# Lainshower/debiasing-multi-modal

Measured on AMD Instinct MI355X. Metric: images/sec (embed+adapter step), CLIP-RN50 224px bs=1024, higher is better.
Workload: dtype f32; 1 GPU; CLIP-RN50 224px encode_image + adapter(1024-128-1024) CE/SGD step, 1024 images/GPU, global batch 1024 (the metric's configuration, CLIP-RN50 224px bs=1024 on one GPU); global_batch=1024, batch_per_gpu=1024, parallelism=dp1, collective=none

## Files before the change

debiasing-multi-modal_amd/_lib.py:

```python
import ctypes
import glob
import os
import subprocess
from ctypes import c_float, c_int, c_int64, c_size_t, c_void_p

_HERE = os.path.dirname(os.path.abspath(__file__))
CSRC = os.path.join(_HERE, "csrc")
LIB_PATH = os.environ.get("DBMM_LIB") or os.path.join(_HERE, "libdbmm_hip.so")
INCLUDE = os.path.join(os.path.dirname(_HERE), "include")

_lib = None


def sources():
    return sorted(glob.glob(os.path.join(CSRC, "*.hip")))


KERNEL_SOURCES = (
    ("igemm_", ("igemm_f32.hip", "igemm_epilogue.inc", "common.h")),
    ("bottleneck_chain_kernel", ("bottleneck_chain.hip", "common.h")),
    ("bottleneck_chain8_kernel", ("bottleneck_chain8.hip", "common.h")),
    ("conv3x3_c32_kernel", ("conv_patch.hip", "common.h")),
    ("gemm_pair_8ph_kernel", ("gemm_pair_8ph.hip", "common.h")),
    ("conv3x3_halo8", ("conv3x3_halo8.hip", "conv3x3_halo8_epilogue.inc", "common.h")),
# ... 82 lines not shown
    "dbmm_bottleneck_chain_x2": [_P, _P, _P, _I, _P, _P, _P, _P, _P, _P, _P, _I, _P, _P, _P, _P, _L, _L, _L, _L, _L, _L, _P],
    "dbmm_bottleneck_chain_dual_x2": [_P, _P, _P, _I, _P, _P, _P, _P, _P, _P, _P, _P, _P, _I, _P, _P, _P, _P, _L, _L, _L, _L, _L, _P],
    "dbmm_gemm_f16": [_P, _L, _P, _L, _P, _P, _L, _P, _L, _L, _L, _L, _I, _P],
    "dbmm_gemm_f16_ws": [_P, _L, _P, _L, _P, _P, _L, _P, _L, _L, _L, _L, _I, _P, _Z, _P],
    "dbmm_mha_core_f16": [_P, _P, _L, _L, _L, _L, _I, _P],
    "dbmm_layernorm_f16": [_P, _L, _P, _P, _P, _L, _L, _L, _F, _P],
    "dbmm_conv1x1_bn_act_f16": [_P, _P, _P, _P, _P, _P, _L, _L, _L, _I, _P],
    "dbmm_conv1x1_bn_act_f16_ws": [_P, _P, _P, _P, _P, _P, _L, _L, _L, _I, _P, _Z, _P],
    "dbmm_conv1x1_dual_bn_act_f16": [_P, _P, _P, _P, _P, _P, _P, _P, _L, _L, _L, _L, _I, _P],
    "dbmm_bottleneck_chain_f16": [_P, _P, _P, _P, _P, _P, _P, _P, _P, _P, _L, _L, _L, _L, _P],
    "dbmm_bottleneck_chain_pool_f16": [_P, _P, _P, _P, _P, _P, _P, _P, _P, _P, _P, _L, _L, _L, _L, _L, _L, _P],
    "dbmm_bottleneck_chain_dual_f16": [_P, _P, _P, _P, _P, _P, _P, _P, _P, _P, _P, _P, _L, _L, _L, _L, _L, _P],
    "dbmm_conv3x3_bn_relu_f16": [_P, _P, _P, _P, _P, _L, _L, _L, _L, _L, _I, _P],
    "dbmm_conv_stem_s2_f16": [_P, _I, _P, _P, _P, _L, _L, _L, _L, _P],
    "dbmm_conv1x1_res_pool_f16": [_P, _P, _P, _P, _P, _P, _P, _L, _L, _L, _L, _L, _P],
    "dbmm_conv_stem_s2_bn_f16": [_P, _I, _P, _P, _P, _P, _L, _L, _L, _L, _P],
    "dbmm_avgpool2_f16": [_P, _P, _L, _L, _L, _L, _P],
    "dbmm_im2col_patch_f16": [_P, _I, _P, _L, _L, _L, _L, _P],
    "dbmm_vit_tokens_f16": [_P, _P, _P, _P, _L, _L, _L, _P],
    "dbmm_embed_gather_f16": [_P, _P, _P, _P, _L, _L, _L, _L, _P],
    "dbmm_gather_eot_f16": [_P, _P, _P, _L, _L, _L, _P],
    "dbmm_cast_f32_f16": [_P, _P, _L, _P],
    "dbmm_conv3x3_c32_bn_relu_x2": [_P, _P, _P, _I, _P, _P, _P, _P, _L, _L, _L, _L, _L, _I, _P],
    "dbmm_bottleneck_block_chain_x2": [_P, _P, _P, _I, _P, _P, _P, _I, _P, _P, _P, _P, _P, _P, _P, _P, _P, _P, _I, _P, _P, _P, _P,
                                       _L, _L, _L, _L, _L, _L, _P],
    "dbmm_gemm_bias_act_x3": [_P, _L, _P, _P, _L, _P, _P, _L, _P, _L, _L, _L, _L, _F, _I, _P, _Z, _P],
    "dbmm_gemm_batched": [_P, _L, _L, _I, _P, _L, _L, _I, _P, _L, _P, _L, _L, _L, _L, _L, _L, _F, _I, _P],
    "dbmm_gemm_pair_8ph": [_P, _L, _P, _P, _I, _L, _P, _P, _P, _L, _P, _L, _P, _L, _L, _L, _F, _I, _P],
    "dbmm_conv_stem_s2": [_P, _P, _P, _P, _P, _L, _L, _L, _L, _P],
    "dbmm_avgpool2d": [_P, _P, _L, _L, _L, _L, _L, _P],
    "dbmm_workspace_bytes_attnpool": [_L, _L, _L],
    "dbmm_attnpool": [_P, _P, _P, _P, _P, _P, _P, _P, _P, _L, _L, _L, _L, _L, _P, _Z, _P],
    "dbmm_attnpool_x": [_P, _I, _P, _P, _P, _P, _P, _P, _P, _P, _L, _L, _L, _L, _L, _P, _Z, _P],
    "dbmm_layernorm": [_P, _L, _P, _P, _P, _L, _L, _L, _F, _P, _P],
    "dbmm_mha_core": [_P, _P, _L, _L, _L, _L, _I, _P],
    "dbmm_mha_core_x2": [_P, _P, _P, _L, _L, _L, _L, _I, _P],
    "dbmm_embed_gather": [_P, _P, _P, _P, _L, _L, _L, _L, _P],
    "dbmm_im2col_patch": [_P, _P, _P, _L, _L, _L, _P],
    "dbmm_vit_tokens": [_P, _P, _P, _P, _L, _L, _L, _P],
    "dbmm_gather_eot": [_P, _P, _P, _L, _L, _L, _P],
    "dbmm_bn1d_stats": [_P, _L, _L, _F, _F, _P, _P, _P, _P, _P, _P],
    "dbmm_bn1d_relu": [_P, _P, _P, _P, _P, _P, _L, _L, _I, _F, _P],
    "dbmm_adapter_fwd": [_P] * 15 + [_L, _L, _L, _I, _F, _F, _P],
    "dbmm_workspace_bytes_adapter_bwd": [_L, _L, _L],
    "dbmm_adapter_bwd": [_P] * 15 + [_L, _L, _L, _P, _Z, _P],
    "dbmm_text_colnorm": [_P, _P, _L, _L, _P],
# ... 93 lines not shown
```

debiasing-multi-modal_amd/clip/model.py:

```python
import os
import re
from collections import OrderedDict
from typing import Tuple, Union

import numpy as np
import torch
from torch import nn

from .. import ops



class _ConvW(nn.Module):
    def __init__(self, cin, cout, k):
        super().__init__()
        self.weight = nn.Parameter(torch.empty(cout, cin, k, k))


class _BNParams(nn.Module):
    def __init__(self, c):
        super().__init__()
        self.weight = nn.Parameter(torch.ones(c))
        self.bias = nn.Parameter(torch.zeros(c))
        self.register_buffer("running_mean", torch.zeros(c))
# ... 50 lines not shown
        super().__init__()
        self.positional_embedding = nn.Parameter(torch.randn(spacial_dim ** 2 + 1, embed_dim) / embed_dim ** 0.5)
        self.k_proj = _LinearW(embed_dim, embed_dim)
        self.q_proj = _LinearW(embed_dim, embed_dim)
        self.v_proj = _LinearW(embed_dim, embed_dim)
        self.c_proj = _LinearW(embed_dim, output_dim or embed_dim)
        self.num_heads = num_heads


def _fold_bn(conv_w, bn):
    s = bn.weight.double() / torch.sqrt(bn.running_var.double() + bn.eps)
    w = conv_w.double() * s.reshape(-1, 1, 1, 1)
    b = bn.bias.double() - bn.running_mean.double() * s
    return w, b


def _conv_bn(conv, bn):
    w, b = _fold_bn(conv.weight, bn)
    scale = bn.weight.detach().double() / torch.sqrt(bn.running_var.detach().double() + bn.eps)
    return _pack_conv(w, b, raw=conv.weight.detach().float(), scale=scale)


_PLAN_OPTIONS = {"conv_split": ("f16", ("f16", "bf16", "off")), "conv_k_order": ("chunk32", ("chunk32", "tap")),
                 "fuse_ds": (1, (0, 1)), "fuse_chain": (1, (0, 1)), "fuse_conv2": (1, (0, 1)), "seam_pool": (2, (0, 1, 2))}
_opt = {}
_opt_version = [0]


def set_plan_option(name, value):
    default, allowed = _PLAN_OPTIONS[name]
    if isinstance(default, int):
        value = int(value)
    if value not in allowed:
        raise ValueError(f"plan option {name}: {value!r} not in {allowed}")
    old = _opt.get(name, default)
    _opt[name] = value
    _opt_version[0] += 1
    return old


def plan_option(name):
    return _opt[name]


for _name in _PLAN_OPTIONS:
    set_plan_option(_name, os.environ.get("DBMM_" + _name.upper(), _PLAN_OPTIONS[_name][0]))

# ... 188 lines not shown
        out = ops.attnpool(x, a["pos"], a["wq"], a["bq"], a["wkv"], a["bkv"], a["wc"], a["bc"], self.attnpool.num_heads)
        out = out.to(torch.float16)
        return (out, stages) if return_stages else out

    def rounds_fp32_images_itself(self):
        return (self.conv1.weight.dtype == torch.float16 and self._f16_eligible()
                and all(b.stride in (1, 2) for li in (1, 2, 3, 4) for b in getattr(self, f"layer{li}")))

    @torch.no_grad()
    def forward(self, x, return_stages=False):
        if self.conv1.weight.dtype == torch.float16:
            if self._f16_eligible() and all(b.stride in (1, 2) for li in (1, 2, 3, 4) for b in getattr(self, f"layer{li}")):
                return self.forward_f16(x, return_stages)
            if not return_stages:
                return self.forward(x, return_stages=True)[0].to(torch.float16)
        if self._plan is not None and self._plan_key != self._param_key():
            self._plan = None
        P = self._plan or self._compile()
        x = x.float().contiguous()
        n_slots = 3 + 4 * len(P["blocks"])
        amax = torch.zeros(n_slots, device=x.device, dtype=torch.float32)
        slot = [1]
        track = _opt["conv_split"] == "f16"
        x = ops.conv_stem_s2(x, *P["stem1"], y_absmax=amax[0:1] if track else None)

        def conv(t, t_am, c, res, k, pad, act, pool=1, keep_full=False):
            y_am = amax[slot[0]:slot[0] + 1] if track else None; slot[0] += 1
            y = ops.conv_bn_act(t, c["w"], c["b"], res, k, k, 1, pad, act, c["wl"], w_planes=c["p3"],
                                w_planes_f16=c["ph"], w_exp=c["we"], x_absmax=t_am, y_absmax=y_am, out_scale=c["sc"],
                                pool=pool, keep_full=keep_full)
            return y, y_am

        x, am = conv(x, amax[0:1] if track else None, P["stem2"], None, 3, 1, ops.ACT_RELU)
        x, am = conv(x, am, P["stem3"], None, 3, 1, ops.ACT_RELU, pool=2)
        stages = {"stem": x}
        blocks = P["blocks"]
        x_pooled = None
        y1_next = None
        bi = 0
        for li in (1, 2, 3, 4):
            for _ in getattr(self, f"layer{li}"):
                e = blocks[bi]; bi += 1
                if y1_next is not None:
                    (out, oam), y1_next = y1_next, None
                else:
                    out, oam = conv(x, am, e["c1"], None, 1, 0, ops.ACT_RELU)
                nxt = blocks[bi] if bi < len(blocks) else None
                if (e["stride"] == 1 and track and _opt["fuse_chain"] and _opt["fuse_conv2"] and nxt is not None and nxt["stride"] == 1
                        and all(c["sc"] is not None and c["ph"] is not None for c in (e["c2"], e["c3"], nxt["c1"]))
                        and ("ds" not in e or ("dual" in e and _opt["fuse_ds"]))):
                    ndsl = 3 if "ds" in e else 2
                    x_am, y1_am = amax[slot[0] + 1:slot[0] + 2], amax[slot[0] + ndsl:slot[0] + ndsl + 1]
                    dual = dict(a2=x, a2_absmax=am, ds=e["ds"], ratio=e["dual"]["ratio"], bias=e["dual"]["bias"]) if "ds" in e else None
                    r = ops.bottleneck_block_chain(out, oam, e["c2"], e["c3"], nxt["c1"], residual=None if dual else x, dual=dual,
                                                   x_absmax=x_am, y1n_absmax=y1_am)
                    if r is not None:
# ... 343 lines not shown
```

debiasing-multi-modal_amd/csrc/common.h:

```cpp
#pragma once
#include <hip/hip_runtime.h>
#include <stdint.h>
#include <type_traits>
#include "../../include/dbmm.h"

typedef float f32x4 __attribute__((ext_vector_type(4)));
typedef float f32x16 __attribute__((ext_vector_type(16)));

#define DBMM_CHECK_LAUNCH()                      \
    do {                                         \
        hipError_t e__ = hipGetLastError();      \
        if (e__ != hipSuccess) return (int)e__;  \
    } while (0)

enum DbmmOpt {
    OPT_IGEMM_EPI_DIRECT, OPT_IGEMM_FAST, OPT_IGEMM_STREAMK, OPT_IGEMM_X3, OPT_IGEMM_X2, OPT_IGEMM_X2_BK, OPT_IGEMM_BK,
    OPT_IGEMM_HALO, OPT_IGEMM_HALO_POOL, OPT_IGEMM_BN256, OPT_IGEMM_BN256_KXK, OPT_GEMM_8PH, OPT_F16_8PH, OPT_F16_BN256,
    OPT_STEM_MFMA, OPT_MHA_VALU, OPT_CONV_PATCH, OPT_MHA_X2, OPT_ADAPTER_STEP_FUSED, OPT_CONV1X1_STREAM, OPT_CONV1X1_8PH, OPT_CHAIN8, OPT_CONV1X1_BN256, OPT_TAIL_SPLIT, OPT_HALO8, OPT_DUAL_8PH, OPT_MHA_SHORT, OPT_F16_CONV_8PH, OPT_CONV1X1_RES_STREAM, OPT_LINEAR_STEP_ONE_LAUNCH_MAX_B, DBMM_OPT_COUNT
};
int dbmm_opt(int id);

int dbmm_conv3x3_halo8(const float* x, const float* x_absmax, const void* w_plane_f16, int w_exp, const float* out_scale, const float* bias,
                       float* y, float* y_absmax, int64_t B, int64_t H, int64_t W, int64_t Cin, int64_t Cout, int act, int pool, int split,
                       void* workspace, size_t workspace_bytes, void* stream);

int dbmm_gemm_pair_8ph_ws(const float* a, int64_t lda, const float* a_absmax, const void* w_plane_f16, int w_exp, int64_t ldw,
                          const float* out_scale, const float* bias, const float* residual, int64_t ldr, float* c, int64_t ldc,
                          float* c_absmax, int64_t M, int64_t N, int64_t K, float alpha, int act, void* workspace, size_t workspace_bytes, void* stream);
int dbmm_gemm_dual_pair_8ph(const float* a, int64_t lda, const float* a_absmax, const void* w_plane_f16, int w_exp, int64_t ldw, int64_t K,
                            const float* out_scale, const float* a2, int64_t lda2, const float* a2_absmax, const void* w2_plane_f16, int64_t ldw2,
                            int64_t K2, const float* ratio, const float* bias, float* c, int64_t ldc, float* c_absmax, int64_t M, int64_t N, int act,
                            void* stream);

static inline int dbmm_cut_slices(int rem, int trips) {
    if (rem <= 0 || rem > 128) return 0;
    int S = 256 / rem;
    S = S < trips ? S : trips;
    S = S < 16 ? S : 16;
    return S >= 2 ? S : 0;
}

// ... 26 lines not shown
```

debiasing-multi-modal_amd/csrc/conv_patch.hip:

```cpp
#include <stdlib.h>
#include "common.h"

namespace {

typedef _Float16 f16x8 __attribute__((ext_vector_type(8)));
typedef unsigned short u16;
typedef unsigned int u32x2 __attribute__((ext_vector_type(2)));
typedef unsigned int u32x4 __attribute__((ext_vector_type(4)));

constexpr unsigned OOR = 0x80000000u;
constexpr long long EXT_LIM = 0x7FFFFFF0LL;
constexpr int TR = 4, TC = 28;
constexpr int PR = TR + 2, PC = TC + 2, PPX = PR * PC;
constexpr int CIN = 32, KTOT = 9 * CIN;
constexpr int WROW = KTOT + 8;

struct PatchP {
    const float* x; const float* x_absmax;
    const u16* w; int w_exp; const float* sc; const float* bias;
    float* y; float* y_absmax;
    int B, H, W, tiles_w, tiles_h, n_tiles;
};

__device__ __forceinline__ int scale_exp(float amax) {
    const unsigned b = __float_as_uint(amax) & 0x7fffffffu;
    int s = b ? 13 - ((int)(b >> 23) - 127) : 0;
    return s < -60 ? -60 : (s > 60 ? 60 : s);
}
__device__ __forceinline__ float pow2f(int e) { return __uint_as_float((unsigned)(e + 127) << 23); }

__device__ __forceinline__ void split2h_pair(float x0, float x1, float sc, unsigned& hi, unsigned& lo) {
#if defined(__HIP_DEVICE_COMPILE__)
    asm("v_fma_mixlo_f16 %0, %1, %2, 0" : "=v"(hi) : "v"(x0), "v"(sc));
    asm("v_fma_mixhi_f16 %0, %1, %2, 0" : "+v"(hi) : "v"(x1), "v"(sc));
    asm("v_fma_mixlo_f16 %0, %1, %2, -%3 op_sel_hi:[0,0,1]" : "=v"(lo) : "v"(x0), "v"(sc), "v"(hi));
    asm("v_fma_mixhi_f16 %0, %1, %2, -%3 op_sel:[0,0,1] op_sel_hi:[0,0,1]" : "+v"(lo) : "v"(x1), "v"(sc), "v"(hi));
#else
    (void)x0; (void)x1; (void)sc; hi = lo = 0;
#endif
}

__device__ __forceinline__ __amdgpu_buffer_rsrc_t desc(const void* base, long long total, long long shift) {
    long long ext = total - shift;
    ext = ext < 0 ? 0 : (ext > EXT_LIM ? EXT_LIM : ext);
    return __builtin_amdgcn_make_buffer_rsrc((void*)((const char*)base + shift), 0, (int)ext, 0x00020000);
}
__device__ __forceinline__ int pswz(int row) { return (row >> 2) & 3; }

template <int N, int POOL>
__global__ __launch_bounds__(256, N == 32 ? 3 : 2) void conv3x3_c32_kernel(const PatchP p) {
    constexpr int TN = N / 32, NLD = (PPX * 8 + 255) / 256;
    constexpr int PCL = POOL ? 40 : PC, PLN = PR * PCL * 32;
    __shared__ __attribute__((aligned(16))) u16 lds[N * WROW + 2 * PLN];
    u16* Wl = lds;
    u16* Pl = lds + N * WROW;
    const int tid = threadIdx.x, lane = tid & 63, wave = tid >> 6;
    const int fr = lane & 31, fh = lane >> 5;

    for (int i = tid; i < N * (KTOT / 8); i += 256) {
        const int n = i / (KTOT / 8), c = i - n * (KTOT / 8);
        *(u32x4*)(Wl + n * WROW + c * 8) = *(const u32x4*)(p.w + (size_t)n * KTOT + c * 8);
    }
    const int s_a = scale_exp(*p.x_absmax);
    const float a_sc = pow2f(s_a), acc_scale = pow2f(-s_a - p.w_exp);
    float sv[TN], bv[TN];
#pragma unroll
    for (int j = 0; j < TN; ++j) { sv[j] = p.sc[j * 32 + fr] * acc_scale; bv[j] = p.bias[j * 32 + fr]; }

    const int ml = wave * 32 + fr;
    int a_dy, a_c;
    bool a_ok;
    if (POOL) { const int o = ml >> 2, q = ml & 3; a_dy = 2 * (o / 14) + (q >> 1); a_c = 2 * (o % 14) + (q & 1); a_ok = ml < TR * TC; }
    else { a_dy = wave; a_c = fr; a_ok = fr < TC; }
    const int a_row0 = a_ok ? a_dy * PCL + a_c : 0;

    const long long img_bytes = (long long)p.H * p.W * CIN * 4;
    f32x4 pre[NLD];
    auto tile_coords = [&](int tile, int& b, int& h0, int& w0) {
        const int tw = tile % p.tiles_w, r = tile / p.tiles_w;
        b = r / p.tiles_h; h0 = (r - b * p.tiles_h) * TR; w0 = tw * TC;
    };
    auto load_patch = [&](int tile) {
        int b, h0, w0;
        tile_coords(tile, b, h0, w0);
        const __amdgpu_buffer_rsrc_t rs = desc(p.x, (long long)p.B * img_bytes, (long long)b * img_bytes);
#pragma unroll
        for (int k = 0; k < NLD; ++k) {
            const int idx = tid + 256 * k, i = idx >> 3, quad = idx & 7;
            const int py = i / PC, px = i - py * PC, h = h0 - 1 + py, w = w0 - 1 + px;
            const bool ok = i < PPX && h >= 0 && h < p.H && w >= 0 && w < p.W;
            pre[k] = __builtin_bit_cast(f32x4, __builtin_amdgcn_raw_buffer_load_b128(
                rs, ok ? (unsigned)((h * p.W + w) * (CIN * 4) + quad * 16) : OOR, 0, 0));
        }
    };
    auto store_patch = [&]() {
#pragma unroll
        for (int k = 0; k < NLD; ++k) {
            const int idx = tid + 256 * k, i = idx >> 3, quad = idx & 7;
            if (i < PPX) {
                unsigned hp[2], lp[2];
#pragma unroll
                for (int j = 0; j < 2; ++j) split2h_pair(pre[k][2 * j], pre[k][2 * j + 1], a_sc, hp[j], lp[j]);
                const int py = i / PC, row = py * PCL + (i - py * PC);
                const int off = row * 32 + (((quad >> 1) ^ pswz(row)) << 3) + ((quad & 1) << 2);
                *(u32x2*)(Pl + off) = (u32x2){hp[0], hp[1]};
                *(u32x2*)(Pl + PLN + off) = (u32x2){lp[0], lp[1]};
            }
        }
    };

    float amax = 0.f;
    int tile = blockIdx.x;
    if (tile < p.n_tiles) load_patch(tile);
    for (; tile < p.n_tiles; tile += gridDim.x) {
        store_patch();
        __syncthreads();
        if (tile + (int)gridDim.x < p.n_tiles) load_patch(tile + gridDim.x);

        f32x16 acc[TN];
#pragma unroll
        for (int j = 0; j < TN; ++j)
#pragma unroll
            for (int r = 0; r < 16; ++r) acc[j][r] = 0.f;
#pragma unroll
        for (int tap = 0; tap < 9; ++tap) {
            const int row = a_row0 + (tap / 3) * PCL + (tap % 3);
#pragma unroll
            for (int ks = 0; ks < 2; ++ks) {
                const int aoff = row * 32 + (((2 * ks + fh) ^ pswz(row)) << 3);
                const u32x4 ah = *(const u32x4*)(Pl + aoff), al = *(const u32x4*)(Pl + PLN + aoff);
                u32x4 wf[TN];
#pragma unroll
                for (int j = 0; j < TN; ++j) wf[j] = *(const u32x4*)(Wl + (j * 32 + fr) * WROW + tap * 32 + (2 * ks + fh) * 8);
#pragma unroll
                for (int j = 0; j < TN; ++j)
                    acc[j] = __builtin_amdgcn_mfma_f32_32x32x16_f16(__builtin_bit_cast(f16x8, al), __builtin_bit_cast(f16x8, wf[j]), acc[j], 0, 0, 0);
#pragma unroll
                for (int j = 0; j < TN; ++j)
                    acc[j] = __builtin_amdgcn_mfma_f32_32x32x16_f16(__builtin_bit_cast(f16x8, ah), __builtin_bit_cast(f16x8, wf[j]), acc[j], 0, 0, 0);
            }
// ... 6 lines not shown
            const long long base_px = ((long long)b * Hp + (h0 >> 1)) * Wp + (w0 >> 1);
            const __amdgpu_buffer_rsrc_t rs = desc(p.y, tot, base_px * N * 4);
#pragma unroll
            for (int t = 0; t < 4; ++t) {
                const int o = wave * 8 + 2 * t + fh;
                const unsigned off = o < 28 ? (unsigned)(((o / 14) * Wp + (o % 14)) * (N * 4) + fr * 4) : OOR;
#pragma unroll
                for (int j = 0; j < TN; ++j) {
                    float v[4];
#pragma unroll
                    for (int q = 0; q < 4; ++q) v[q] = fmaxf(fmaf(acc[j][4 * t + q], sv[j], bv[j]), 0.f);
                    const float s = (((v[0] + v[1]) + v[2]) + v[3]) * 0.25f;
                    __builtin_amdgcn_raw_buffer_store_b32(__builtin_bit_cast(unsigned, s), rs, off, (unsigned)(j * 128), 0);
                    if (o < 28) amax = fmaxf(amax, fmaxf(fmaxf(v[0], v[1]), fmaxf(v[2], v[3])));
                }
            }
        } else {
            const long long tot = (long long)p.B * p.H * p.W * N * 4;
            const long long base_px = ((long long)b * p.H + h0) * p.W + w0;
            const __amdgpu_buffer_rsrc_t rs = desc(p.y, tot, base_px * N * 4);
#pragma unroll
            for (int r = 0; r < 16; ++r) {
                const int c = (r & 3) + 8 * (r >> 2) + 4 * fh, dy = wave;
                const bool m_ok = c < TC;
                const unsigned off = m_ok ? (unsigned)((dy * p.W + c) * (N * 4) + fr * 4) : OOR;
#pragma unroll
                for (int j = 0; j < TN; ++j) {
                    const float v = fmaxf(fmaf(acc[j][r], sv[j], bv[j]), 0.f);
                    __builtin_amdgcn_raw_buffer_store_b32(__builtin_bit_cast(unsigned, v), rs, off, (unsigned)(j * 128), 0);
                    if (m_ok) amax = fmaxf(amax, v);
                }
            }
        }
        __syncthreads();
    }
    if (p.y_absmax) {
        amax = wave_max(amax);
        float* red = (float*)Pl;
        if (lane == 0) red[wave] = amax;
        __syncthreads();
        if (tid == 0) {
            const float m = fmaxf(fmaxf(red[0], red[1]), fmaxf(red[2], red[3]));
            if (m > *(volatile const float*)p.y_absmax) atomicMax((unsigned*)p.y_absmax, __float_as_uint(m));
        }
    }
}

}

extern "C" int dbmm_conv3x3_c32_bn_relu_x2(const float* x, const float* x_absmax, const void* w_plane_f16, int w_exp,
                                           const float* scale, const float* bias, float* y, float* y_absmax, int64_t B, int64_t H,
                                           int64_t W, int64_t Cin, int64_t Cout, int pool, void* stream) {
    if (!x || !x_absmax || !w_plane_f16 || !scale || !bias || !y) return DBMM_E_ARG;
    if (B <= 0 || H <= 0 || W <= 0 || (pool != 0 && pool != 2)) return DBMM_E_SHAPE;
    if (Cin != CIN || (Cout != 32 && Cout != 64) || (H % TR) || (W % TC) || w_exp < -40 || w_exp > 40) return DBMM_E_UNSUPPORTED;
    if (H * W * CIN * 4 >= EXT_LIM || B * (H / TR) * (W / TC) > INT32_MAX) return DBMM_E_UNSUPPORTED;
    if (!dbmm_aligned16(x) || !dbmm_aligned16(w_plane_f16) || !dbmm_aligned16(y)) return DBMM_E_ALIGN;
    PatchP p{};
    p.x = x; p.x_absmax = x_absmax; p.w = (const u16*)w_plane_f16; p.w_exp = w_exp; p.sc = scale; p.bias = bias;
    p.y = y; p.y_absmax = y_absmax; p.B = (int)B; p.H = (int)H; p.W = (int)W;
    p.tiles_w = (int)(W / TC); p.tiles_h = (int)(H / TR); p.n_tiles = (int)(B * p.tiles_h * p.tiles_w);
    const int per_cu = Cout == 32 ? 3 : 2;
    const int grid = p.n_tiles < 256 * per_cu ? p.n_tiles : 256 * per_cu;
    hipStream_t s = (hipStream_t)stream;
    if (Cout == 32) {
        if (pool) hipLaunchKernelGGL((conv3x3_c32_kernel<32, 1>), dim3(grid), dim3(256), 0, s, p);
        else hipLaunchKernelGGL((conv3x3_c32_kernel<32, 0>), dim3(grid), dim3(256), 0, s, p);
    } else {
        if (pool) hipLaunchKernelGGL((conv3x3_c32_kernel<64, 1>), dim3(grid), dim3(256), 0, s, p);
        else hipLaunchKernelGGL((conv3x3_c32_kernel<64, 0>), dim3(grid), dim3(256), 0, s, p);
    }
    DBMM_CHECK_LAUNCH();
    return DBMM_OK;
}
```

debiasing-multi-modal_amd/csrc/options.hip:

```cpp
#include <atomic>
#include <ctype.h>
#include <stdlib.h>
#include <string.h>
#include "common.h"

namespace {

struct OptDef { const char* name; int def; };
const OptDef kOpts[DBMM_OPT_COUNT] = {
    {"igemm_epi_direct", 1},
    {"igemm_fast", 1},
    {"igemm_streamk", 1},
    {"igemm_x3", 1},
    {"igemm_x2", 1},
    {"igemm_x2_bk", 32},
    {"igemm_bk", 0},
    {"igemm_halo", 1},
    {"igemm_halo_pool", 2},
    {"igemm_bn256", 1},
    {"igemm_bn256_kxk", 1},
    {"gemm_8ph", 1},
    {"f16_8ph", 1},
    {"f16_bn256", 1},
    {"stem_mfma", 1},
    {"mha_valu", 0},
    {"conv_patch", 1},
    {"mha_x2", 1},
    {"adapter_step_fused", 1},
    {"conv1x1_stream", 1},
    {"conv1x1_8ph", 1},
    {"chain8", 0},
    {"conv1x1_bn256", 0},
    {"tail_split", 1},
    {"halo8", 1},
    {"dual_8ph", 1},
    {"mha_short", 1},
    {"f16_conv_8ph", 1},
    {"conv1x1_res_stream", 1},
    {"linear_step_one_launch_max_b", 512},
};

std::atomic<int> g_val[DBMM_OPT_COUNT];

struct Seed {
    Seed() {
        for (int i = 0; i < DBMM_OPT_COUNT; ++i) {
            char env[64] = "DBMM_";
            size_t n = strlen(env);
            for (const char* c = kOpts[i].name; *c && n + 1 < sizeof(env); ++c) env[n++] = (char)toupper((unsigned char)*c);
            env[n] = 0;
            const char* e = getenv(env);
            g_val[i].store(e ? atoi(e) : kOpts[i].def, std::memory_order_relaxed);
        }
    }
} g_seed;

int find(const char* name) {
    if (!name) return -1;
    for (int i = 0; i < DBMM_OPT_COUNT; ++i)
        if (!strcmp(name, kOpts[i].name)) return i;
    return -1;
}
// ... 19 lines not shown
```

debiasing-multi-modal_amd/ops.py:

```python
import ctypes
import math
import os

import torch

from . import _lib
from ._lib import check, ptr, require_cuda, stream

ACT_NONE, ACT_RELU, ACT_QUICKGELU = 0, 1, 2


class DbmmUnsupported(_lib.DbmmError):
    """a wrapper's C entry answered DBMM_E_UNSUPPORTED (no kernel for this valid request)"""


def set_option(name, value):
    old = get_option(name)
    check(_lib.lib().dbmm_set_option(name.encode(), int(value)), f"set_option({name})")
    return old


def get_option(name):
    v = ctypes.c_int()
    check(_lib.lib().dbmm_get_option(name.encode(), ctypes.byref(v)), f"get_option({name})")
# ... 379 lines not shown
                                                 ptr(a2), ptr(a2_absmax), ptr(ds["ph"]), ptr(ratio), ptr(x), ptr(x_absmax),
                                                 ptr(c1["ph"]), int(c1["we"]), ptr(c1["sc"]), ptr(c1["b"]), ptr(y1),
                                                 ptr(y1_absmax), M, K, K2, N, P, stream())
    if rc == _lib.E_UNSUPPORTED:
        return None
    check(rc, "bottleneck_chain_dual_x2")
    t.__exit__(None, None, None)
    return x, y1


def conv_stem_s2(x_nchw, w, bias, y_absmax=None):
    require_cuda(x_nchw, w)
    _f32c(x_nchw); _f32c(w)
    B, C, H, W = x_nchw.shape
    if C != 3:
        raise _lib.DbmmError("stem conv expects 3 input channels")
    Cout = w.shape[-1]
    y = _empty((B, (H - 1) // 2 + 1, (W - 1) // 2 + 1, Cout), device=x_nchw.device, dtype=torch.float32)
    check(_lib.lib().dbmm_conv_stem_s2(ptr(x_nchw), ptr(w), ptr(bias), ptr(y), ptr(y_absmax), B, H, W, Cout, stream()),
          "conv_stem_s2")
    return y


def avgpool2d(x, k):
    require_cuda(x)
    _f32c(x)
    B, H, W, C = x.shape
    y = _empty((B, H // k, W // k, C), device=x.device, dtype=torch.float32)
    check(_lib.lib().dbmm_avgpool2d(ptr(x), ptr(y), B, H, W, C, k, stream()), "avgpool2d")
    return y


def attnpool(x, pos, wq, bq, wkv, bkv, wc, bc, heads):
    require_cuda(x)
    if x.dtype != torch.float16:
        _f32c(x)
    elif not x.is_contiguous():
        raise _lib.DbmmError("attnpool: expected a contiguous tensor")
    B, H, W, C = x.shape
    HW = H * W
    Dout = wc.shape[0]
    if tuple(pos.shape) != (HW + 1, C):
        raise RuntimeError(f"attnpool: positional embedding {tuple(pos.shape)} does not match a {H} x {W} x {C} feature map "
                           f"(expected ({HW + 1}, {C})): the input resolution differs from the one the model was built for")
    if (tuple(wq.shape) != (C, C) or tuple(wkv.shape) != (2 * C, C) or wc.shape[1] != C or bq.numel() != C or bkv.numel() != 2 * C
            or bc.numel() != Dout):
# ... 829 lines not shown
```

include/dbmm.h:

```cpp
#ifndef DBMM_H
#define DBMM_H

#include <stddef.h>
#include <stdint.h>

#ifdef __cplusplus
extern "C" {
#endif

#define DBMM_OK 0
#define DBMM_E_SHAPE (-1)
#define DBMM_E_ALIGN (-2)
#define DBMM_E_WORKSPACE (-3)
#define DBMM_E_ARG (-4)
#define DBMM_E_UNSUPPORTED (-5)

#define DBMM_WL_TAP_MAJOR 0
#define DBMM_WL_CHUNK_MAJOR 1
#define DBMM_WL_CHUNK32_MAJOR 2

#define DBMM_ACT_NONE 0
#define DBMM_ACT_RELU 1
#define DBMM_ACT_QUICKGELU 2

// ... 45 lines not shown
int dbmm_conv_bn_act_x2(const float* x, const float* x_absmax, const float* w, const void* w_planes_f16,
                        int w_planes, int w_exp, const float* out_scale, const float* bias,
                        const float* residual, float* y, float* y_full, float* y_absmax,
                        int64_t B, int64_t H, int64_t W, int64_t Cin, int64_t Cout, int64_t KH, int64_t KW,
                        int64_t stride, int64_t pad, int act, int pool, int w_layout, void* workspace,
                        size_t workspace_bytes, void* stream);

int dbmm_gemm_bias_act_x2(const float* a, int64_t lda, const float* a_absmax, const float* w,
                          const void* w_planes_f16, int w_planes, int w_exp, int64_t ldw,
                          const float* out_scale, const float* bias, const float* residual, int64_t ldr,
                          float* c, int64_t ldc, float* c_absmax, int64_t M, int64_t N, int64_t K, float alpha,
                          int act, void* workspace, size_t workspace_bytes, void* stream);

int dbmm_gemm_dual_bn_act_x2(const float* a, int64_t lda, const float* a_absmax, const void* w_plane_f16,
                             int w_exp, int64_t ldw, int64_t K, const float* out_scale, const float* a2,
                             int64_t lda2, const float* a2_absmax, const void* w2_plane_f16, int64_t ldw2,
                             int64_t K2, const float* ratio, const float* bias, float* c, int64_t ldc,
                             float* c_absmax, int64_t M, int64_t N, int act, void* workspace,
                             size_t workspace_bytes, void* stream);

int dbmm_conv3x3_c32_bn_relu_x2(const float* x, const float* x_absmax, const void* w_plane_f16, int w_exp,
                                const float* scale, const float* bias, float* y, float* y_absmax, int64_t B, int64_t H,
                                int64_t W, int64_t Cin, int64_t Cout, int pool, void* stream);

int dbmm_bottleneck_chain_x2(const float* y2, const float* y2_absmax, const void* w3_plane_f16, int w3_exp,
                             const float* scale3, const float* bias3, const float* residual, float* x_out,
                             float* x_pooled, float* x_absmax, const void* w1_plane_f16, int w1_exp,
                             const float* scale1, const float* bias1, float* y1_out, float* y1_absmax,
                             int64_t B, int64_t Ho, int64_t Wo, int64_t K, int64_t N, int64_t P, void* stream);

int dbmm_bottleneck_chain_dual_x2(const float* y2, const float* y2_absmax, const void* w3_plane_f16, int w3_exp,
                                  const float* scale3, const float* bias, const float* a2, const float* a2_absmax,
                                  const void* wd_plane_f16, const float* ratio, float* x_out, float* x_absmax,
                                  const void* w1_plane_f16, int w1_exp, const float* scale1, const float* bias1,
                                  float* y1_out, float* y1_absmax, int64_t M, int64_t K, int64_t K2, int64_t N,
                                  int64_t P, void* stream);

int dbmm_bottleneck_block_chain_x2(const float* y1, const float* y1_absmax, const void* w2_plane_f16, int w2_exp,
                                   const float* scale2, const float* bias2, const void* w3_plane_f16, int w3_exp,
                                   const float* scale3, const float* bias3, const float* residual, const float* a2,
                                   const float* a2_absmax, const void* wd_plane_f16, const float* ratio, float* x_out,
                                   float* x_absmax, const void* w1_plane_f16, int w1_exp, const float* scale1,
                                   const float* bias1, float* y1_out, float* y1_out_absmax, int64_t B, int64_t H,
                                   int64_t W, int64_t K, int64_t N, int64_t P, void* stream);

int dbmm_gemm_pair_8ph(const float* a, int64_t lda, const float* a_absmax, const void* w_plane_f16, int w_exp, int64_t ldw,
// ... 211 lines not shown
```

Measured before the change: 35630 images/sec.

## Fuse stem conv1 (stride-2, 3-channel) into stem conv2 patch kernel

Adds a variant of the 3x3 c32 patch conv kernel that reads the raw NCHW image tile, computes stem conv1 (3->32, stride 2, folded BN, ReLU) on the fly with split-f16 MFMA, and feeds the result straight into conv2's LDS patch. This removes the launch and the full write/read of conv1's 112x112x32 activation. In exchange it recomputes conv1 halo pixels per tile and derives the f16 split scale per tile rather than globally, which adds per-tile syncs and may shift numerics slightly.

```diff
diff --git a/debiasing-multi-modal_amd/_lib.py b/debiasing-multi-modal_amd/_lib.py
--- a/debiasing-multi-modal_amd/_lib.py
+++ b/debiasing-multi-modal_amd/_lib.py
@@ -128,6 +128,7 @@
     "dbmm_gather_eot_f16": [_P, _P, _P, _L, _L, _L, _P],
     "dbmm_cast_f32_f16": [_P, _P, _L, _P],
     "dbmm_conv3x3_c32_bn_relu_x2": [_P, _P, _P, _I, _P, _P, _P, _P, _L, _L, _L, _L, _L, _I, _P],
+    "dbmm_conv_stem12_c32_x2": [_P, _P, _P, _P, _I, _P, _P, _P, _P, _L, _L, _L, _P],
     "dbmm_bottleneck_block_chain_x2": [_P, _P, _P, _I, _P, _P, _P, _I, _P, _P, _P, _P, _P, _P, _P, _P, _P, _P, _I, _P, _P, _P, _P,
                                        _L, _L, _L, _L, _L, _L, _P],
     "dbmm_gemm_bias_act_x3": [_P, _L, _P, _P, _L, _P, _P, _L, _P, _L, _L, _L, _L, _F, _I, _P, _Z, _P],
diff --git a/debiasing-multi-modal_amd/clip/model.py b/debiasing-multi-modal_amd/clip/model.py
--- a/debiasing-multi-modal_amd/clip/model.py
+++ b/debiasing-multi-modal_amd/clip/model.py
@@ -96,7 +96,8 @@
 
 
 _PLAN_OPTIONS = {"conv_split": ("f16", ("f16", "bf16", "off")), "conv_k_order": ("chunk32", ("chunk32", "tap")),
-                 "fuse_ds": (1, (0, 1)), "fuse_chain": (1, (0, 1)), "fuse_conv2": (1, (0, 1)), "seam_pool": (2, (0, 1, 2))}
+                 "fuse_ds": (1, (0, 1)), "fuse_chain": (1, (0, 1)), "fuse_conv2": (1, (0, 1)), "seam_pool": (2, (0, 1, 2)),
+                 "stem_fuse": (1, (0, 1))}
 _opt = {}
 _opt_version = [0]
 
@@ -331,7 +332,14 @@
         amax = torch.zeros(n_slots, device=x.device, dtype=torch.float32)
         slot = [1]
         track = _opt["conv_split"] == "f16"
-        x = ops.conv_stem_s2(x, *P["stem1"], y_absmax=amax[0:1] if track else None)
+        img, x = x, None
+        s1, s2 = P["stem1"], P["stem2"]
+        if (track and _opt["stem_fuse"] and s1[0].shape[-1] == 32 and s2["ph"] is not None and s2["sc"] is not None
+                and img.shape[2] % 2 == 0 and img.shape[3] % 2 == 0):
+            x = ops.conv_stem12(img, s1[0], s1[1], s2, y_absmax=amax[1:2])
+        fused12 = x is not None
+        if not fused12:
+            x = ops.conv_stem_s2(img, *P["stem1"], y_absmax=amax[0:1] if track else None)
 
         def conv(t, t_am, c, res, k, pad, act, pool=1, keep_full=False):
             y_am = amax[slot[0]:slot[0] + 1] if track else None; slot[0] += 1
@@ -340,7 +348,10 @@
                                 pool=pool, keep_full=keep_full)
             return y, y_am
 
-        x, am = conv(x, amax[0:1] if track else None, P["stem2"], None, 3, 1, ops.ACT_RELU)
+        if fused12:
+            am = amax[1:2]; slot[0] += 1
+        else:
+            x, am = conv(x, amax[0:1] if track else None, P["stem2"], None, 3, 1, ops.ACT_RELU)
         x, am = conv(x, am, P["stem3"], None, 3, 1, ops.ACT_RELU, pool=2)
         stages = {"stem": x}
         blocks = P["blocks"]
diff --git a/debiasing-multi-modal_amd/csrc/common.h b/debiasing-multi-modal_amd/csrc/common.h
--- a/debiasing-multi-modal_amd/csrc/common.h
+++ b/debiasing-multi-modal_amd/csrc/common.h
@@ -16,7 +16,7 @@
 enum DbmmOpt {
     OPT_IGEMM_EPI_DIRECT, OPT_IGEMM_FAST, OPT_IGEMM_STREAMK, OPT_IGEMM_X3, OPT_IGEMM_X2, OPT_IGEMM_X2_BK, OPT_IGEMM_BK,
     OPT_IGEMM_HALO, OPT_IGEMM_HALO_POOL, OPT_IGEMM_BN256, OPT_IGEMM_BN256_KXK, OPT_GEMM_8PH, OPT_F16_8PH, OPT_F16_BN256,
-    OPT_STEM_MFMA, OPT_MHA_VALU, OPT_CONV_PATCH, OPT_MHA_X2, OPT_ADAPTER_STEP_FUSED, OPT_CONV1X1_STREAM, OPT_CONV1X1_8PH, OPT_CHAIN8, OPT_CONV1X1_BN256, OPT_TAIL_SPLIT, OPT_HALO8, OPT_DUAL_8PH, OPT_MHA_SHORT, OPT_F16_CONV_8PH, OPT_CONV1X1_RES_STREAM, OPT_LINEAR_STEP_ONE_LAUNCH_MAX_B, DBMM_OPT_COUNT
+    OPT_STEM_MFMA, OPT_MHA_VALU, OPT_CONV_PATCH, OPT_MHA_X2, OPT_ADAPTER_STEP_FUSED, OPT_CONV1X1_STREAM, OPT_CONV1X1_8PH, OPT_CHAIN8, OPT_CONV1X1_BN256, OPT_TAIL_SPLIT, OPT_HALO8, OPT_DUAL_8PH, OPT_MHA_SHORT, OPT_F16_CONV_8PH, OPT_CONV1X1_RES_STREAM, OPT_LINEAR_STEP_ONE_LAUNCH_MAX_B, OPT_STEM_FUSE, DBMM_OPT_COUNT
 };
 int dbmm_opt(int id);
 
diff --git a/debiasing-multi-modal_amd/csrc/conv_patch.hip b/debiasing-multi-modal_amd/csrc/conv_patch.hip
--- a/debiasing-multi-modal_amd/csrc/conv_patch.hip
+++ b/debiasing-multi-modal_amd/csrc/conv_patch.hip
@@ -20,7 +20,10 @@
     const u16* w; int w_exp; const float* sc; const float* bias;
     float* y; float* y_absmax;
     int B, H, W, tiles_w, tiles_h, n_tiles;
+    const float* img; const float* w1; const float* b1; int IH, IW;
 };
+constexpr int WR = 2 * PR + 1, WC = 2 * PC + 1, WIN = 3 * WR * WC;
+constexpr int WIN_LDS = (WIN + 3) / 4 * 4 + 8;
 
 __device__ __forceinline__ int scale_exp(float amax) {
     const unsigned b = __float_as_uint(amax) & 0x7fffffffu;
@@ -47,25 +50,29 @@
 }
 __device__ __forceinline__ int pswz(int row) { return (row >> 2) & 3; }
 
-template <int N, int POOL>
+template <int N, int POOL, int SRC = 0>
 __global__ __launch_bounds__(256, N == 32 ? 3 : 2) void conv3x3_c32_kernel(const PatchP p) {
-    constexpr int TN = N / 32, NLD = (PPX * 8 + 255) / 256;
+    static_assert(!SRC || (N == 32 && !POOL), "the image-sourced patch serves conv2 of the stem only");
+    constexpr int TN = N / 32, NLD = SRC ? (3 * WR + 3) / 4 : (PPX * 8 + 255) / 256;
     constexpr int PCL = POOL ? 40 : PC, PLN = PR * PCL * 32;
-    __shared__ __attribute__((aligned(16))) u16 lds[N * WROW + 2 * PLN];
+    __shared__ __attribute__((aligned(16))) u16 lds[N * WROW + 2 * PLN + (SRC ? 2 * WIN_LDS : 0)];
     u16* Wl = lds;
     u16* Pl = lds + N * WROW;
+    float* Iw = (float*)(lds + N * WROW + 2 * PLN);
+    float* wred = Iw + WIN_LDS - 8;
     const int tid = threadIdx.x, lane = tid & 63, wave = tid >> 6;
     const int fr = lane & 31, fh = lane >> 5;
+    const int wu = __builtin_amdgcn_readfirstlane(wave);
 
     for (int i = tid; i < N * (KTOT / 8); i += 256) {
         const int n = i / (KTOT / 8), c = i - n * (KTOT / 8);
         *(u32x4*)(Wl + n * WROW + c * 8) = *(const u32x4*)(p.w + (size_t)n * KTOT + c * 8);
     }
-    const int s_a = scale_exp(*p.x_absmax);
-    const float a_sc = pow2f(s_a), acc_scale = pow2f(-s_a - p.w_exp);
-    float sv[TN], bv[TN];
-#pragma unroll
-    for (int j = 0; j < TN; ++j) { sv[j] = p.sc[j * 32 + fr] * acc_scale; bv[j] = p.bias[j * 32 + fr]; }
+    int s_a = SRC ? 0 : scale_exp(*p.x_absmax);
+    float a_sc = pow2f(s_a), acc_scale = pow2f(-s_a - p.w_exp);
+    float sv0[TN], sv[TN], bv[TN];
+#pragma unroll
+    for (int j = 0; j < TN; ++j) { sv0[j] = p.sc[j * 32 + fr]; sv[j] = sv0[j] * acc_scale; bv[j] = p.bias[j * 32 + fr]; }
 
     const int ml = wave * 32 + fr;
     int a_dy, a_c;
@@ -75,7 +82,7 @@
     const int a_row0 = a_ok ? a_dy * PCL + a_c : 0;
 
     const long long img_bytes = (long long)p.H * p.W * CIN * 4;
-    f32x4 pre[NLD];
+    typename std::conditional<SRC != 0, float, f32x4>::type pre[NLD];
     auto tile_coords = [&](int tile, int& b, int& h0, int& w0) {
         const int tw = tile % p.tiles_w, r = tile / p.tiles_w;
         b = r / p.tiles_h; h0 = (r - b * p.tiles_h) * TR; w0 = tw * TC;
@@ -83,6 +90,20 @@
     auto load_patch = [&](int tile) {
         int b, h0, w0;
         tile_coords(tile, b, h0, w0);
+        if constexpr (SRC) {
+            const long long ib = 3LL * p.IH * p.IW * 4;
+            const __amdgpu_buffer_rsrc_t rs = desc(p.img, (long long)p.B * ib, (long long)b * ib);
+            const int iw = 2 * w0 - 3 + lane;
+            const bool col_ok = lane < WC && iw >= 0 && iw < p.IW;
+#pragma unroll
+            for (int k = 0; k < NLD; ++k) {
+                const int row = 4 * k + wu, c = row / WR, ih = 2 * h0 - 3 + row - c * WR;
+                const bool row_ok = row < 3 * WR && ih >= 0 && ih < p.IH;
+                pre[k] = __builtin_bit_cast(float, __builtin_amdgcn_raw_buffer_load_b32(
+                    rs, row_ok && col_ok ? (unsigned)(iw * 4) : OOR, row_ok ? (unsigned)((c * p.IH + ih) * p.IW * 4) : 0u, 0));
+            }
+            return;
+        } else {
         const __amdgpu_buffer_rsrc_t rs = desc(p.x, (long long)p.B * img_bytes, (long long)b * img_bytes);
 #pragma unroll
         for (int k = 0; k < NLD; ++k) {
@@ -92,8 +113,15 @@
             pre[k] = __builtin_bit_cast(f32x4, __builtin_amdgcn_raw_buffer_load_b128(
                 rs, ok ? (unsigned)((h * p.W + w) * (CIN * 4) + quad * 16) : OOR, 0, 0));
         }
+        }
     };
     auto store_patch = [&]() {
+        if constexpr (SRC) {
+#pragma unroll
+            for (int k = 0; k < NLD; ++k)
+                if (lane < WC && 4 * k + wu < 3 * WR) Iw[(4 * k + wu) * WC + lane] = pre[k];
+            return;
+        } else {
 #pragma unroll
         for (int k = 0; k < NLD; ++k) {
             const int idx = tid + 256 * k, i = idx >> 3, quad = idx & 7;
@@ -105,6 +133,91 @@
                 const int off = row * 32 + (((quad >> 1) ^ pswz(row)) << 3) + ((quad & 1) << 2);
                 *(u32x2*)(Pl + off) = (u32x2){hp[0], hp[1]};
                 *(u32x2*)(Pl + PLN + off) = (u32x2){lp[0], lp[1]};
+            }
+        }
+        }
+    };
+
+    auto slot_tap = [](int f, int t, int& kh, int& kw, int& c) -> bool {
+        int pr;
+        if (t < 9) { kh = f; pr = t; }
+        else { kh = 2; pr = f ? t - 2 : t - 9; if (pr > 8) { kh = kw = c = 0; return false; } }
+        kw = pr / 3; c = pr - kw * 3;
+        return true;
+    };
+    unsigned w1h[2][4], w1l[2][4];
+    float b1v = 0.f;
+    int e_w = 0;
+    if constexpr (SRC) {
+        float wv[16], wmax = 0.f;
+#pragma unroll
+        for (int t = 0; t < 16; ++t) {
+            int kh0, kw0, c0, kh1, kw1, c1;
+            const bool v0 = slot_tap(0, t, kh0, kw0, c0), v1 = slot_tap(1, t, kh1, kw1, c1);
+            const int k = fh ? (kh1 * 3 + kw1) * 3 + c1 : (kh0 * 3 + kw0) * 3 + c0;
+            wv[t] = (fh ? v1 : v0) ? p.w1[k * 32 + fr] : 0.f;
+            wmax = fmaxf(wmax, fabsf(wv[t]));
+        }
+        e_w = scale_exp(wave_max(wmax));
+        const float sc = pow2f(e_w);
+#pragma unroll
+        for (int ks = 0; ks < 2; ++ks)
+#pragma unroll
+            for (int q = 0; q < 4; ++q) split2h_pair(wv[ks * 8 + 2 * q], wv[ks * 8 + 2 * q + 1], sc, w1h[ks][q], w1l[ks][q]);
+        b1v = p.b1[fr];
+    }
+    auto conv1_block = [&](int blk, int h0, int w0, float (&v)[16]) {
+        const int pi = blk * 32 + fr, py = pi / PC, px = pi - py * PC;
+        const bool row_ok = pi < PPX;
+        const int base = row_ok ? 2 * py * WC + 2 * px : 0;
+        const int ph = h0 - 1 + py, pw = w0 - 1 + px;
+        const unsigned okb = (unsigned)__builtin_amdgcn_ballot_w64(row_ok && ph >= 0 && ph < p.H && pw >= 0 && pw < p.W);
+        const unsigned okm = fh ? okb >> 4 : okb;
+        const int baseA = base + fh * WC, baseB = base + fh * (WR * WC + 2);
+        float xv[16], amax = 0.f;
+#pragma unroll
+        for (int t = 0; t < 16; ++t) {
+            int kh0, kw0, c0, kh1, kw1, c1;
+            const bool v0 = slot_tap(0, t, kh0, kw0, c0), v1 = slot_tap(1, t, kh1, kw1, c1);
+            const int off0 = (c0 * WR + kh0) * WC + kw0, off1 = (c1 * WR + kh1) * WC + kw1;
+            static_assert(WR * WC + 2 == (1 * WR + 2) * WC + 2 - (0 * WR + 2) * WC, "slot map");
+            (void)off1;
+            const float x = Iw[(t < 9 ? baseA : (v1 ? baseB : base)) + (t < 9 ? off0 - kh0 * WC : off0)];
+            xv[t] = (row_ok && (fh ? v1 : v0)) ? x : 0.f;
+            amax = fmaxf(amax, fabsf(xv[t]));
+        }
+        const int e_a = scale_exp(wave_max(amax));
+        const float sc = pow2f(e_a), osc = pow2f(-e_a - e_w);
+        unsigned ah[2][4], al[2][4];
+#pragma unroll
+        for (int ks = 0; ks < 2; ++ks)
+#pragma unroll
+            for (int q = 0; q < 4; ++q) split2h_pair(xv[ks * 8 + 2 * q], xv[ks * 8 + 2 * q + 1], sc, ah[ks][q], al[ks][q]);
+        auto frag = [](const unsigned (&u)[4]) { return __builtin_bit_cast(f16x8, (u32x4){u[0], u[1], u[2], u[3]}); };
+        f32x16 acc;
+#pragma unroll
+        for (int r = 0; r < 16; ++r) acc[r] = 0.f;
+#pragma unroll
+        for (int ks = 0; ks < 2; ++ks) {
+            acc = __builtin_amdgcn_mfma_f32_32x32x16_f16(frag(al[ks]), frag(w1h[ks]), acc, 0, 0, 0);
+            acc = __builtin_amdgcn_mfma_f32_32x32x16_f16(frag(ah[ks]), frag(w1l[ks]), acc, 0, 0, 0);
+        }
+#pragma unroll
+        for (int ks = 0; ks < 2; ++ks)
+            acc = __builtin_amdgcn_mfma_f32_32x32x16_f16(frag(ah[ks]), frag(w1h[ks]), acc, 0, 0, 0);
+#pragma unroll
+        for (int r = 0; r < 16; ++r) v[r] = ((okm >> ((r & 3) + 8 * (r >> 2))) & 1u) ? fmaxf(fmaf(acc[r], osc, b1v), 0.f) : 0.f;
+    };
+    auto split_block = [&](int blk, const float (&v)[16]) {
+#pragma unroll
+        for (int r = 0; r < 16; ++r) {
+            const int q = blk * 32 + (r & 3) + 8 * (r >> 2) + 4 * fh;
+            if (q < PPX) {
+                const float xs = v[r] * a_sc;
+                const _Float16 h = (_Float16)xs, l = (_Float16)(xs - (float)h);
+                const int off = q * 32 + (((fr >> 3) ^ pswz(q)) << 3) + (fr & 7);
+                Pl[off] = __builtin_bit_cast(u16, h);
+                Pl[PLN + off] = __builtin_bit_cast(u16, l);
             }
         }
     };
@@ -116,6 +229,31 @@
         store_patch();
         __syncthreads();
         if (tile + (int)gridDim.x < p.n_tiles) load_patch(tile + gridDim.x);
+        if constexpr (SRC) {
+            int b_, h0_, w0_;
+            tile_coords(tile, b_, h0_, w0_);
+            float c1a[16], c1b[16];
+            conv1_block(wu, h0_, w0_, c1a);
+            float tmax = 0.f;
+#pragma unroll
+            for (int r = 0; r < 16; ++r) tmax = fmaxf(tmax, c1a[r]);
+            if (wave < 2) {
+                conv1_block(wu + 4, h0_, w0_, c1b);
+#pragma unroll
+                for (int r = 0; r < 16; ++r) tmax = fmaxf(tmax, c1b[r]);
+            }
+            tmax = wave_max(tmax);
+            float* tr = wred + 4 * ((tile / (int)gridDim.x) & 1);
+            if (lane == 0) tr[wave] = tmax;
+            __syncthreads();
+            s_a = scale_exp(fmaxf(fmaxf(tr[0], tr[1]), fmaxf(tr[2], tr[3])));
+            a_sc = pow2f(s_a); acc_scale = pow2f(-s_a - p.w_exp);
+#pragma unroll
+            for (int j = 0; j < TN; ++j) sv[j] = sv0[j] * acc_scale;
+            split_block(wu, c1a);
+            if (wave < 2) split_block(wu + 4, c1b);
+            __syncthreads();
+        }
 
         f32x16 acc[TN];
 #pragma unroll
@@ -168,7 +306,7 @@
 #pragma unroll
             for (int r = 0; r < 16; ++r) {
                 const int c = (r & 3) + 8 * (r >> 2) + 4 * fh, dy = wave;
-                const bool m_ok = c < TC;
+                const bool m_ok = c < TC && (!SRC || (w0 + c < p.W && h0 + dy < p.H));
                 const unsigned off = m_ok ? (unsigned)((dy * p.W + c) * (N * 4) + fr * 4) : OOR;
 #pragma unroll
                 for (int j = 0; j < TN; ++j) {
@@ -178,10 +316,11 @@
                 }
             }
         }
-        __syncthreads();
+        if constexpr (!SRC) __syncthreads();
     }
     if (p.y_absmax) {
         amax = wave_max(amax);
+        if constexpr (SRC) __syncthreads();
         float* red = (float*)Pl;
         if (lane == 0) red[wave] = amax;
         __syncthreads();
@@ -219,3 +358,24 @@
     DBMM_CHECK_LAUNCH();
     return DBMM_OK;
 }
+
+extern "C" int dbmm_conv_stem12_c32_x2(const float* x_nchw, const float* w1, const float* bias1, const void* w2_plane_f16, int w2_exp,
+                                       const float* scale2, const float* bias2, float* y, float* y_absmax, int64_t B, int64_t H, int64_t W,
+                                       void* stream) {
+    if (!x_nchw || !w1 || !bias1 || !w2_plane_f16 || !scale2 || !bias2 || !y) return DBMM_E_ARG;
+    if (B <= 0 || H <= 0 || W <= 0) return DBMM_E_SHAPE;
+    if (w2_exp < -40 || w2_exp > 40 || 3 * H * W * 8 >= EXT_LIM) return DBMM_E_UNSUPPORTED;
+    const int64_t Ho = (H - 1) / 2 + 1, Wo = (W - 1) / 2 + 1;
+    const int64_t th = (Ho + TR - 1) / TR, tw = (Wo + TC - 1) / TC;
+    if (Ho * Wo * CIN * 4 >= EXT_LIM || B * th * tw > INT32_MAX) return DBMM_E_UNSUPPORTED;
+    if (!dbmm_aligned16(w2_plane_f16) || !dbmm_aligned16(y)) return DBMM_E_ALIGN;
+    PatchP p{};
+    p.img = x_nchw; p.w1 = w1; p.b1 = bias1; p.IH = (int)H; p.IW = (int)W;
+    p.w = (const u16*)w2_plane_f16; p.w_exp = w2_exp; p.sc = scale2; p.bias = bias2;
+    p.y = y; p.y_absmax = y_absmax; p.B = (int)B; p.H = (int)Ho; p.W = (int)Wo;
+    p.tiles_w = (int)tw; p.tiles_h = (int)th; p.n_tiles = (int)(B * th * tw);
+    const int grid = p.n_tiles < 256 * 3 ? p.n_tiles : 256 * 3;
+    hipLaunchKernelGGL((conv3x3_c32_kernel<32, 0, 1>), dim3(grid), dim3(256), 0, (hipStream_t)stream, p);
+    DBMM_CHECK_LAUNCH();
+    return DBMM_OK;
+}
diff --git a/debiasing-multi-modal_amd/csrc/options.hip b/debiasing-multi-modal_amd/csrc/options.hip
--- a/debiasing-multi-modal_amd/csrc/options.hip
+++ b/debiasing-multi-modal_amd/csrc/options.hip
@@ -38,6 +38,7 @@
     {"f16_conv_8ph", 1},
     {"conv1x1_res_stream", 1},
     {"linear_step_one_launch_max_b", 512},
+    {"stem_fuse", 1},
 };
 
 std::atomic<int> g_val[DBMM_OPT_COUNT];
diff --git a/debiasing-multi-modal_amd/ops.py b/debiasing-multi-modal_amd/ops.py
--- a/debiasing-multi-modal_amd/ops.py
+++ b/debiasing-multi-modal_amd/ops.py
@@ -425,6 +425,35 @@
     return y
 
 
+def conv_stem12(x_nchw, w1, bias1, c2, y_absmax=None):
+    require_cuda(x_nchw, w1, bias1)
+    _f32c(x_nchw); _f32c(w1); _f32c(bias1)
+    if x_nchw.dim() != 4 or x_nchw.shape[1] != 3:
+        raise _lib.DbmmError("stem conv expects an NCHW batch with 3 input channels")
+    if w1.numel() != 27 * 32 or w1.shape[-1] != 32:
+        raise RuntimeError(f"conv_stem12: conv1 weight {tuple(w1.shape)} where the kernel indexes [3][3][3][32]")
+    _sized("conv_stem12 bias1", bias1, 32)
+    ph, sc, b2 = c2.get("ph"), c2.get("sc"), c2.get("b")
+    if (ph is None or sc is None or b2 is None or ph.shape[0] != 1 or tuple(ph.shape[1:]) != (32, 288)
+            or c2.get("wl", WL_TAP_MAJOR) not in (WL_TAP_MAJOR, WL_CHUNK32_MAJOR) or not get_option("stem_fuse") or not get_option("conv_patch")):
+        return None
+    _sized("conv_stem12 scale2", sc, 32); _sized("conv_stem12 bias2", b2, 32); _sized("conv_stem12 y_absmax", y_absmax, 1)
+    B, _, H, W = x_nchw.shape
+    Ho, Wo = (H - 1) // 2 + 1, (W - 1) // 2 + 1
+    y = _empty((B, Ho, Wo, 32), device=x_nchw.device, dtype=torch.float32)
+    global _chain_tag
+    _chain_tag = "conv3x3_c32_kernel<32, 0>"
+    t = _Timed(B * Ho * Wo, 32, 9 * 32 + 27, -1, 0, 4 * (x_nchw.numel() + y.numel()) + 2 * 32 * 288 + 4 * 28 * 32)
+    t.__enter__()
+    rc = _lib.lib().dbmm_conv_stem12_c32_x2(ptr(x_nchw), ptr(w1), ptr(bias1), ptr(ph), int(c2["we"]), ptr(sc), ptr(b2), ptr(y),
+                                            ptr(y_absmax), B, H, W, stream())
+    if rc in (_lib.E_UNSUPPORTED, _lib.E_ALIGN):
+        return None
+    check(rc, "conv_stem12_c32_x2")
+    t.__exit__(None, None, None)
+    return y
+
+
 def avgpool2d(x, k):
     require_cuda(x)
     _f32c(x)
diff --git a/include/dbmm.h b/include/dbmm.h
--- a/include/dbmm.h
+++ b/include/dbmm.h
@@ -91,6 +91,10 @@
 int dbmm_conv3x3_c32_bn_relu_x2(const float* x, const float* x_absmax, const void* w_plane_f16, int w_exp,
                                 const float* scale, const float* bias, float* y, float* y_absmax, int64_t B, int64_t H,
                                 int64_t W, int64_t Cin, int64_t Cout, int pool, void* stream);
+
+int dbmm_conv_stem12_c32_x2(const float* x_nchw, const float* w1, const float* bias1, const void* w2_plane_f16, int w2_exp,
+                            const float* scale2, const float* bias2, float* y, float* y_absmax, int64_t B, int64_t H, int64_t W,
+                            void* stream);
 
 int dbmm_bottleneck_chain_x2(const float* y2, const float* y2_absmax, const void* w3_plane_f16, int w3_exp,
                              const float* scale3, const float* bias3, const float* residual, float* x_out,
```

Result: no change. 35620 images/sec (-0.0%).
